# kleinzcy/speech_signal_processing

Hardware: AMD Instinct MI355X
Metric: MFCC frames/s (one fused pass: framing .. DCT + delta + delta-delta, 39-d) (higher is better)
Workload: dtype f32; 1 GPU; configs[1]: 100000 x 3 s synthetic 16 kHz utterances per GPU, 39-d MFCC (+delta+delta-delta), 400/160/512, 24 mel; utterances_per_gpu=100000, frames_per_gpu=29800000, d_out=39, parallelism=utterance-sharded x1, world_size_observed=1

## Files before the change

speech_signal_processing_amd/csrc/cplx.hpp:

```cpp
#pragma once
#include <hip/hip_runtime.h>

namespace ssp {

typedef float v2f __attribute__((ext_vector_type(2)));
typedef float v4f __attribute__((ext_vector_type(4)));
typedef __attribute__((address_space(3))) void* lds_ptr_t;


__device__ __forceinline__ v2f swap(v2f z) { return v2f{z.y, z.x}; }
__device__ __forceinline__ v2f xx(v2f z) { return v2f{z.x, z.x}; }
__device__ __forceinline__ v2f yy(v2f z) { return v2f{z.y, z.y}; }
__device__ __forceinline__ v2f add_neg_i(v2f t, v2f u) { return __builtin_elementwise_fma(swap(u), v2f{1.f, -1.f}, t); }
__device__ __forceinline__ v2f sub_neg_i(v2f t, v2f u) { return __builtin_elementwise_fma(swap(u), v2f{-1.f, 1.f}, t); }
__device__ __forceinline__ v2f cmulc(v2f z, float c, float s) {
    return __builtin_elementwise_fma(yy(z), v2f{-s, c}, xx(z) * v2f{c, s});
}
__device__ __forceinline__ v2f cmul(v2f z, v2f w) {
    v2f t, r;
    asm("v_pk_mul_f32 %0, %1, %2 op_sel_hi:[0,1]" : "=v"(t) : "v"(z), "v"(w));
    asm("v_pk_fma_f32 %0, %1, %2, %3 op_sel:[1,1,0] op_sel_hi:[1,0,1] neg_lo:[0,1,0]"
        : "=v"(r) : "v"(z), "v"(w), "v"(t));
    return r;
}
__device__ __forceinline__ v2f cmul_negi(v2f z, v2f w) {
    v2f t, r;
    asm("v_pk_mul_f32 %0, %1, %2 op_sel:[1,0] op_sel_hi:[1,1]" : "=v"(t) : "v"(z), "v"(w));
    asm("v_pk_fma_f32 %0, %1, %2, %3 op_sel:[0,1,0] op_sel_hi:[0,0,1] neg_hi:[0,1,0]"
        : "=v"(r) : "v"(z), "v"(w), "v"(t));
    return r;
}
__device__ __forceinline__ v2f cmul2(v2f z, v2f w, v2f iw) { return __builtin_elementwise_fma(yy(z), iw, xx(z) * w); }

__device__ __forceinline__ void dft4(v2f& a, v2f& b, v2f& c, v2f& d) {
    const v2f t0 = a + c, t1 = a - c, t2 = b + d, u = b - d;
    a = t0 + t2;
    c = t0 - t2;
    b = add_neg_i(t1, u);
    d = sub_neg_i(t1, u);
}

__device__ __forceinline__ void dft4_d0(v2f& a, v2f& b, v2f& c, v2f& d) {
    const v2f t0 = a + c, t1 = a - c, u = b;
    a = t0 + u;
    c = t0 - u;
    b = add_neg_i(t1, u);
    d = sub_neg_i(t1, u);
}

template <bool TAIL0 = false>
__device__ __forceinline__ void fft16_in(v2f (&z)[16]) {
    constexpr float C1 = 0.92387953251128674f, S1 = 0.38268343236508977f, R = 0.70710678118654752f;
    dft4(z[0], z[4], z[8], z[12]);
#pragma unroll
    for (int n2 = 1; n2 < 4; ++n2) {
        if (TAIL0) dft4_d0(z[n2], z[n2 + 4], z[n2 + 8], z[n2 + 12]);
        else dft4(z[n2], z[n2 + 4], z[n2 + 8], z[n2 + 12]);
    }
    z[5] = cmulc(z[5], C1, -S1);
    z[6] = cmulc(z[6], R, -R);
    z[7] = cmulc(z[7], S1, -C1);
    z[9] = cmulc(z[9], R, -R);
    z[10] = swap(z[10]) * v2f{1.f, -1.f};
    z[11] = cmulc(z[11], -R, -R);
    z[13] = cmulc(z[13], S1, -C1);
    z[14] = cmulc(z[14], -R, -R);
    z[15] = cmulc(z[15], -C1, S1);
#pragma unroll
    for (int k1 = 0; k1 < 4; ++k1) dft4(z[4 * k1], z[4 * k1 + 1], z[4 * k1 + 2], z[4 * k1 + 3]);
    v2f o[16];
#pragma unroll
    for (int k1 = 0; k1 < 4; ++k1)
#pragma unroll
        for (int k2 = 0; k2 < 4; ++k2) o[k1 + 4 * k2] = z[4 * k1 + k2];
#pragma unroll
    for (int i = 0; i < 16; ++i) z[i] = o[i];
}
__device__ __forceinline__ void fft16(v2f (&z)[16]) { fft16_in<false>(z); }

__device__ __forceinline__ void fft8(v2f (&z)[8]) {
    constexpr float R = 0.70710678118654752f;
    dft4(z[0], z[2], z[4], z[6]);
    dft4(z[1], z[3], z[5], z[7]);
    const v2f o0 = z[1], o1 = cmulc(z[3], R, -R), o2 = swap(z[5]) * v2f{1.f, -1.f}, o3 = cmulc(z[7], -R, -R);
    const v2f e0 = z[0], e1 = z[2], e2 = z[4], e3 = z[6];
    z[0] = e0 + o0;
    z[1] = e1 + o1;
    z[2] = e2 + o2;
    z[3] = e3 + o3;
    z[4] = e0 - o0;
    z[5] = e1 - o1;
    z[6] = e2 - o2;
    z[7] = e3 - o3;
}

template <int R>
__device__ __forceinline__ void fft_small(v2f (&z)[R]) {
    if constexpr (R == 2) {
        const v2f a = z[0], b = z[1];
        z[0] = a + b;
        z[1] = a - b;
    } else if constexpr (R == 4) {
        dft4(z[0], z[1], z[2], z[3]);
    } else if constexpr (R == 8) {
        fft8(z);
    } else {
        fft16(z);
    }
}

extern "C" __device__ float ssp_fmul_legacy(float, float) __asm("llvm.amdgcn.fmul.legacy");
__device__ __forceinline__ v2f wmul_edge(v2f y, v2f w) { return v2f{ssp_fmul_legacy(y.x, w.x), ssp_fmul_legacy(y.y, w.y)}; }

__device__ __forceinline__ v2f edge_row_taps(v2f w, int first_tap, int win_len) {
    if (first_tap < win_len && w.x == 0.f) w.x = 1.17549435e-38f;
    if (first_tap + 1 < win_len && w.y == 0.f) w.y = 1.17549435e-38f;
    return w;
}

}
```

speech_signal_processing_amd/csrc/mfcc_stream_kernel.hpp:

```cpp
#pragma once
#include <algorithm>
#include <cmath>
#include <cstdlib>
#include <type_traits>

#include "mfcc.hpp"
#include "cplx.hpp"

namespace ssp {

namespace {
typedef unsigned v2u __attribute__((ext_vector_type(2)));
typedef __attribute__((address_space(3))) const volatile v2f* lds_cv2f_t;
typedef __attribute__((address_space(3))) const volatile float* lds_cvf_t;
typedef __attribute__((address_space(3))) const v2f* lds_c2f_t;
typedef __attribute__((address_space(3))) v4f* lds_4f_t;
constexpr int ZROW = 128;
constexpr int ZFRAME = 16 * ZROW;
constexpr int LM_OFF = 1792;
constexpr int RING_FRAMES = 24;
constexpr int RING_ROW = 64;
constexpr int STREAM_WAVES = 4;
#ifndef SSP_S_PSHIFT
#define SSP_S_PSHIFT 64
#endif
constexpr int PSH = SSP_S_PSHIFT;
static_assert(4 * (256 + 24) + PSH <= LM_OFF - 192, "shifted P row: piece reads must stay below the log-mel rows");
#ifndef SSP_S_NOFLOOR
#define SSP_S_NOFLOOR 1
#endif
#ifndef SSP_S_PUTSC
#define SSP_S_PUTSC 1
#endif
#ifndef SSP_S_AHEAD
#define SSP_S_AHEAD 1
#endif
#ifndef SSP_S_WTAB
#define SSP_S_WTAB 1
#endif
#ifndef SSP_S_LADDR
#define SSP_S_LADDR 1
#endif
constexpr int STREAM_WTAB_N = 39, STREAM_WTAB_BYTES = STREAM_WTAB_N * 8;
constexpr bool stream_wtab(int melv, int ns, int cm, int walk, int geo) { return SSP_S_WTAB && geo >= 2 && !walk && !cm && !(melv >= 4 && ns >= 4); }
#define SSP_STR_(x) #x
#define SSP_STR(x) SSP_STR_(x)

__device__ __forceinline__ float stream_log(const FastArgs& f, float v) {
    return __builtin_amdgcn_logf(fmaxf(v + f.log_add, f.log_max)) * f.log_k;
}

__device__ __forceinline__ float delta_weight(float t, float tp, float Tm1, float half_inv) {
    const float lo = tp <= 0.f ? -1.0e6f : tp;
    const float hi = tp >= Tm1 ? 1.0e6f : tp;
    const float a = fmaxf(lo, t - 2.f), b = fminf(hi, t + 2.f);
    const float cnt = fmaxf(b - a + 1.f, 0.f);
    const float w = cnt * (a + b - 2.f * t) * half_inv;
    return (tp < 0.f || tp > Tm1) ? 0.f : w;
}
}

template <int NZ, int POWER, int PRE, int MELV, int KS, int NS, int OCC, int CM, int WALK, int GEO>
__device__ __forceinline__ void mfcc_stream512_body(const MfccArgs& a, const FastArgs& f, const StreamArgs& sa) {
    static_assert(GEO >= 0 && GEO <= 3 && (GEO == 0 || (NZ == 13 && KS == 6 && MELV != 0)), "fixed geometry: the 400 / 160 / 24-filter family only");
    constexpr bool FIXG = GEO != 0;
    extern __shared__ __attribute__((aligned(16))) char smem[];
    if (WALK && sa.work_counter[1] == 0) return;
    const int tid = threadIdx.x, lane = tid & 63;
    const int wave = __builtin_amdgcn_readfirstlane(tid >> 6);
    const int g = lane >> 4, j = lane & 15;
    constexpr int nc = 13;
    constexpr int mel_ns = NS;

    char* zbuf = smem + wave * sa.wave_bytes;
    float* stage = reinterpret_cast<float*>(zbuf + 4 * ZFRAME);
    char* ring = zbuf + 4 * ZFRAME + sa.stage_bytes;

    v2f wreg[NZ];
#pragma unroll
    for (int n1 = 0; n1 < NZ; ++n1) wreg[n1] = *reinterpret_cast<const v2f*>(a.window + 32 * n1 + 2 * j);
#pragma unroll
    for (int n1 = 0; n1 < NZ; ++n1) wreg[n1] = edge_row_taps(wreg[n1], 32 * n1 + 2 * j, a.win_len);
#ifndef SSP_STREAM_NTW
#define SSP_STREAM_NTW 15
#endif
#ifndef SSP_STREAM_NTW_CM
#define SSP_STREAM_NTW_CM 12
#endif
#ifndef SSP_STREAM_NWP
#define SSP_STREAM_NWP 8
#endif
    constexpr int NTW = OCC >= 3 ? (CM ? SSP_STREAM_NTW_CM : ((MELV <= 3 && NS <= 2) ? SSP_STREAM_NTW : ((MELV >= 4 && NS >= 4) ? 8 : 9))) : 15, NWP = OCC >= 3 ? SSP_STREAM_NWP : 8;
    static_assert(NTW >= 8, "rows above NTW take W^((k1 - 8) j) W^(8 j): W^(8 j) = twr[7] must be resident");
    v2f twr[NTW], wpr[NWP];
#pragma unroll
    for (int k1 = 1; k1 <= NTW; ++k1) twr[k1 - 1] = *reinterpret_cast<const v2f*>(&f.tw16[k1 * 16 + j]);
    float dA[KS];
#pragma unroll
    for (int s = 0; s < KS; ++s) dA[s] = sa.dctA[s * 64 + lane];
#pragma unroll
    for (int i = 0; i < NWP; ++i) wpr[i] = *reinterpret_cast<const v2f*>(&f.wpost[i * 16 + j]);
    constexpr bool DENSE = MELV == 0;
    constexpr int MV = DENSE ? 1 : MELV;
    v4f mw[MV];
    int mofs[MV];
    v2f mk01 = v2f{0.f, 0.f}, mk23 = v2f{0.f, 0.f};
    int mfid = -1;
    v4f dw[DENSE ? 6 : 1][4];
    float dw256[DENSE ? 6 : 1];
    if (DENSE) {
#pragma unroll
        for (int k = 0; k < 6; ++k) {
#pragma unroll
            for (int i = 0; i < 4; ++i) dw[DENSE ? k : 0][i] = *reinterpret_cast<const v4f*>(sa.dense_w + ((size_t)lane * 6 + k) * 20 + 4 * i);
            dw256[DENSE ? k : 0] = sa.dense_w[((size_t)lane * 6 + k) * 20 + 16];
        }
    } else {
#pragma unroll
        for (int i = 0; i < MV; ++i) {
            mw[i] = *reinterpret_cast<const v4f*>(f.pc_w + ((size_t)lane * MV + i) * 4);
            mofs[i] = f.pc_ofs[lane * MV + i];
        }
        mk01 = *reinterpret_cast<const v2f*>(f.pc_mask + lane * 4);
        mk23 = NS > 2 ? *reinterpret_cast<const v2f*>(f.pc_mask + lane * 4 + 2) : v2f{0.f, 0.f};
        mfid = f.pc_fid[lane];
    }

    const int hop = FIXG ? 160 : a.hop;
    const float pre = PRE ? a.preemph : 0.f;
    const float npre = -pre;
    const int slen = FIXG ? 3 * 160 + 32 * 13 : f.slen;
    const int n_piece = (slen + 255) >> 8;
    const bool has_half = (slen & 255) != 0 && (slen & 255) <= 128;
    const int n_full = has_half ? n_piece - 1 : n_piece;
    const int dord = FIXG ? GEO - 1 : a.delta_order;
    const int Dd = FIXG ? nc * GEO : a.d_out;
    const int n_filt = FIXG ? 24 : a.n_filt;
    const int lm_pad = FIXG ? 0 : f.lm_pad;
    const float half_inv = 0.5f * a.delta_inv_denom;
    const uint32_t stage_lds = __builtin_amdgcn_readfirstlane((uint32_t)(uintptr_t)(lds_ptr_t)stage);
    constexpr bool WTAB = FIXG && stream_wtab(MELV, NS, CM, WALK, GEO);
    char* wtab = smem + STREAM_WAVES * sa.wave_bytes;
    if constexpr (WTAB) {
        const float inv = 2.f * half_inv, inv2 = inv * inv;
        const float ds = (float)(lane - 19);
        const float aw = __builtin_fabsf(ds);
        const float w = __builtin_fmaf(aw, __builtin_fmaf(aw * aw, -1.f / 6.f, 37.f / 6.f), -10.f) * inv2;
        if (lane < STREAM_WTAB_N) *reinterpret_cast<v2f*>(wtab + 8 * lane) = v2f{__builtin_fabsf(ds) <= 2.f ? ds * inv : 0.f, aw <= 4.f ? w : 0.f};
        asm volatile("s_waitcnt lgkmcnt(0)" ::: "memory");
    }
    constexpr bool LADDR = FIXG && !WALK && !CM && SSP_S_LADDR;
    int la_dct = 0, la_put = 0, la_pf = 0;
    if constexpr (LADDR) {
        la_dct = (int)(uintptr_t)(lds_ptr_t)(zbuf + (j & 3) * (ZFRAME - 64) + LM_OFF + g * (KS * 4));
        la_put = j < 4 ? (int)(uintptr_t)(lds_ptr_t)(ring + j * RING_ROW + g * 16) : -1;
        la_pf = lane * 16;
        asm volatile("" : "+v"(la_dct), "+v"(la_put), "+v"(la_pf));
    }

#ifdef SSP_S_CLOCK
    const unsigned long long ck0 = __builtin_amdgcn_s_memtime(), rt0 = __builtin_amdgcn_s_memrealtime();
#endif
    uint64_t wm = 0;
    int wblk = blockIdx.x * STREAM_WAVES + wave, wbase = 0;
    constexpr bool AHEAD = FIXG && !WALK && SSP_S_AHEAD;
    typedef int rec_t __attribute__((ext_vector_type(8)));
    int nx_cidx = 0;
    rec_t nx_rec = rec_t{0, 0, 0, 0, 0, 0, 0, 0};
    auto claim_ahead = [&]() {
        const __amdgpu_buffer_rsrc_t rc = __builtin_amdgcn_make_buffer_rsrc(sa.work_counter, 0, 4, 0x00020000);
        int ol = lane;
        asm volatile("" : "+v"(ol));
        const int got = __builtin_amdgcn_raw_ptr_buffer_atomic_add_i32(1, rc, ol == 0 ? 0 : 0x7ffffff0, 0, 0);
        nx_cidx = __builtin_amdgcn_readfirstlane(got);
        const StreamChunkRec* rp = sa.chunk_rec + min(nx_cidx, sa.n_chunks - 1);
        asm volatile("s_load_dwordx8 %0, %1, 0x0\n\ts_waitcnt lgkmcnt(0)" : "=&s"(nx_rec) : "s"(rp) : "memory");
    };
    if constexpr (AHEAD) claim_ahead();
    for (;;) {
        int cidx = 0;
        if constexpr (WALK) {
            bool done = false;
            while (wm == 0) {
                if ((int64_t)wblk * 64 >= sa.n_chunks) {
                    done = true;
                    break;
                }
                const int idx = wblk * 64 + lane;
                const int fl = idx < sa.n_chunks ? sa.redo_flags[idx] : 0;
                wm = __builtin_amdgcn_ballot_w64(fl != 0);
                wbase = wblk * 64;
                wblk += gridDim.x * STREAM_WAVES;
            }
            if (done) break;
            cidx = __builtin_amdgcn_readfirstlane(wbase + __builtin_ctzll(wm));
            wm &= wm - 1;
        } else if constexpr (AHEAD) {
            cidx = nx_cidx;
            if (cidx >= sa.n_chunks) break;
        } else {
            if (lane == 0) cidx = atomicAdd(sa.work_counter, 1);
            cidx = __builtin_amdgcn_readfirstlane(cidx);
            if (cidx >= sa.n_chunks) break;
        }
        MfccChunk ch{};
        int64_t s0, N = 0, f0;
        int T, t0, n, rec_xbytes = 0;
        if constexpr (AHEAD) {
            s0 = (int64_t)(((uint64_t)(uint32_t)nx_rec[1] << 32) | (uint32_t)nx_rec[0]);
            f0 = (int64_t)(((uint64_t)(uint32_t)nx_rec[3] << 32) | (uint32_t)nx_rec[2]);
            rec_xbytes = nx_rec[4];
            T = nx_rec[5];
            t0 = nx_rec[6];
            n = nx_rec[7] & 0xffff;
            ch.pad = nx_rec[7] >> 16;
        } else {
            ch = a.chunks[cidx];
            s0 = a.sample_off[ch.utt];
            N = a.sample_off[ch.utt + 1] - s0;
            f0 = a.frame_off[ch.utt];
            T = __builtin_amdgcn_readfirstlane((int)(a.frame_off[ch.utt + 1] - f0));
            t0 = __builtin_amdgcn_readfirstlane(ch.t0), n = __builtin_amdgcn_readfirstlane(ch.n);
        }
        const int H = dord > 0 ? 4 : 0;
        const int Hlo = dord > 0 ? H + __builtin_amdgcn_readfirstlane(ch.pad) : 0;
        const int ta = max(t0 - Hlo, 0), tb = min(t0 + n + H, T);
        const int R = tb - ta;
        const int nquads = (R + 3) >> 2;
        const int E = t0 + n - ta;
        const int n_steps = (E + 4 + 15) >> 4;
        const int Q = DENSE ? nquads : 4 * n_steps;
        const float Tm1 = (float)(T - 1);

        const uint64_t xaddr = reinterpret_cast<uint64_t>(a.samples + s0);
        const uint32_t xlo = __builtin_amdgcn_readfirstlane((uint32_t)xaddr), xhi = __builtin_amdgcn_readfirstlane((uint32_t)(xaddr >> 32));
        const int xbytes = AHEAD ? rec_xbytes : __builtin_amdgcn_readfirstlane((int)(N * 4));
        const __amdgpu_buffer_rsrc_t rs = __builtin_amdgcn_make_buffer_rsrc(
            reinterpret_cast<float*>(((uint64_t)xhi << 32) | xlo), 0, xbytes, 0x00020000);
        const uint64_t oaddr = reinterpret_cast<uint64_t>(a.out + (size_t)f0 * Dd);
        const uint32_t olo = __builtin_amdgcn_readfirstlane((uint32_t)oaddr), ohi = __builtin_amdgcn_readfirstlane((uint32_t)(oaddr >> 32));
        const __amdgpu_buffer_rsrc_t ro = __builtin_amdgcn_make_buffer_rsrc(
            reinterpret_cast<float*>(((uint64_t)ohi << 32) | olo), 0, __builtin_amdgcn_readfirstlane(T * Dd * 4), 0x00020000);

        auto prefetch = [&](int q) {
            int ol = lane;
            if (FIXG && !LADDR) asm volatile("" : "+v"(ol));
            const int vo = (ta + 4 * q) * hop * 4 + (LADDR ? la_pf : ol * 16);
            const lds_ptr_t lp = (lds_ptr_t)(uintptr_t)stage_lds;
            if (FIXG) {
                __builtin_amdgcn_raw_ptr_buffer_load_lds(rs, lp, 16, vo, 0, 0, 0);
                __builtin_amdgcn_raw_ptr_buffer_load_lds(rs, lp, 16, vo, 0, 1024, 0);
                __builtin_amdgcn_raw_ptr_buffer_load_lds(rs, lp, 16, vo, 0, 2048, 0);
                if (LADDR ? la_pf < 512 : lane < 32) __builtin_amdgcn_raw_ptr_buffer_load_lds(rs, lp, 16, vo, 0, 3072, 0);
                return;
            }
            if (n_full > 0) __builtin_amdgcn_raw_ptr_buffer_load_lds(rs, lp, 16, vo, 0, 0, 0);
            if (n_full > 1) __builtin_amdgcn_raw_ptr_buffer_load_lds(rs, lp, 16, vo, 0, 1024, 0);
            if (n_full > 2) __builtin_amdgcn_raw_ptr_buffer_load_lds(rs, lp, 16, vo, 0, 2048, 0);
            if (n_full > 3) __builtin_amdgcn_raw_ptr_buffer_load_lds(rs, lp, 16, vo, 0, 3072, 0);
            if (n_full > 4) __builtin_amdgcn_raw_ptr_buffer_load_lds(rs, (lds_ptr_t)(uintptr_t)(stage_lds + 4096), 16, vo + 4096, 0, 0, 0);
            if (has_half && lane < 32)
                __builtin_amdgcn_raw_ptr_buffer_load_lds(rs, (lds_ptr_t)(uintptr_t)(stage_lds + n_full * 1024), 16, vo + n_full * 1024, 0, 0, 0);
        };

        {
            float zz = 0.f;
            asm volatile("" : "+v"(zz));
            v4f z4 = v4f{zz, zz, zz, zz};
            *reinterpret_cast<v4f*>(ring + lane * 16) = z4;
            if (lane < (RING_FRAMES * RING_ROW - 1024) / 16) *reinterpret_cast<v4f*>(ring + 1024 + lane * 16) = z4;
        }
        prefetch(0);
        int stores_pending = 0;
        int cm_nf = WALK;
        float cs1[CM ? 3 : 1] = {}, cs2[CM ? 3 : 1] = {};
        float piv = 0.f;

        typedef v2f zarr_t[16];
        typedef v2f pfarr_t[NZ];
        typedef float pmarr_t[PRE ? NZ : 1];
        constexpr int NH = (NZ + 1) / 2;
        auto wait_dma = [&]() {
#ifndef SSP_S_NOWAIT
            if constexpr (FIXG) {
                if (__builtin_expect(stores_pending == 0, 1)) {
                    asm volatile("s_waitcnt vmcnt(0)" ::: "memory");
                } else {
                    int np = stores_pending;
                    asm volatile("" : "+s"(np));
                    if (np == 2 * GEO) asm volatile("s_waitcnt vmcnt(%0)" ::"n"(2 * GEO) : "memory");
                    else asm volatile("s_waitcnt vmcnt(%0)" ::"n"(GEO >= 3 ? 13 : (GEO == 2 ? 9 : 4)) : "memory");
                }
            } else {
                if (stores_pending == 0) asm volatile("s_waitcnt vmcnt(0)" ::: "memory");
                else if (stores_pending == 2) asm volatile("s_waitcnt vmcnt(2)" ::: "memory");
                else if (stores_pending == 4) asm volatile("s_waitcnt vmcnt(4)" ::: "memory");
                else if (stores_pending == 6) asm volatile("s_waitcnt vmcnt(6)" ::: "memory");
                else if (stores_pending == 9) asm volatile("s_waitcnt vmcnt(9)" ::: "memory");
                else asm volatile("s_waitcnt vmcnt(13)" ::: "memory");
            }
#endif
            stores_pending = 0;
        };
        auto stage_read_a = [&](pfarr_t& pf, pmarr_t& pm) {
            const uint32_t sp = stage_lds + (g * hop + 2 * j) * 4;
#pragma unroll
            for (int n1 = 0; n1 < NH; ++n1) {
                pf[n1] = *(lds_cv2f_t)(uintptr_t)(sp + 128 * n1);
#ifdef SSP_S_PM64
                if (PRE) pm[n1] = (*(lds_cv2f_t)(uintptr_t)(sp + 128 * n1 - 8)).y;
#else
                if (PRE) pm[n1] = *(lds_cvf_t)(uintptr_t)(sp + 128 * n1 - 4);
#endif
            }
        };
        auto stage_read_b = [&](pfarr_t& pf, pmarr_t& pm) {
            const uint32_t sp = stage_lds + (g * hop + 2 * j) * 4;
#pragma unroll
            for (int n1 = NH; n1 < NZ; ++n1) {
                pf[n1] = *(lds_cv2f_t)(uintptr_t)(sp + 128 * n1);
#ifdef SSP_S_PM64
                if (PRE) pm[n1] = (*(lds_cv2f_t)(uintptr_t)(sp + 128 * n1 - 8)).y;
#else
                if (PRE) pm[n1] = *(lds_cvf_t)(uintptr_t)(sp + 128 * n1 - 4);
#endif
            }
        };
        auto win_rows = [&](zarr_t& z, pfarr_t& pf, pmarr_t& pm, auto lo_tag, auto hi_tag, auto edge_tag) {
            constexpr int LO = decltype(lo_tag)::value, HI = decltype(hi_tag)::value;
            constexpr int EDGE = decltype(edge_tag)::value;
#pragma unroll
            for (int n1 = LO; n1 < HI; ++n1) {
                if (n1 < NZ) {
                    v2f y = pf[n1 < NZ ? n1 : 0];
                    if (PRE) {
                        const float xm1 = pm[n1 < NZ ? n1 : 0], x0 = y.x, x1 = y.y;
                        y = v2f{__builtin_fmaf(npre, xm1, x0), __builtin_fmaf(npre, x0, x1)};
                    }
                    z[n1] = (EDGE == 1 || (EDGE == 2 && n1 == NZ - 1)) ? wmul_edge(y, wreg[n1 < NZ ? n1 : 0]) : y * wreg[n1 < NZ ? n1 : 0];
                } else {
                    z[n1] = v2f{0.f, 0.f};
                }
            }
        };
        auto window_a = [&](zarr_t& z, pfarr_t& pf, pmarr_t& pm, auto edge_tag) {
            if (PRE) pm[0] = (j == 0) ? pf[0].x : pm[0];
            win_rows(z, pf, pm, std::integral_constant<int, 0>{}, std::integral_constant<int, NH>{}, edge_tag);
        };
        auto window_b = [&](zarr_t& z, pfarr_t& pf, pmarr_t& pm, auto edge_tag) {
            win_rows(z, pf, pm, std::integral_constant<int, NH>{}, std::integral_constant<int, 16>{}, edge_tag);
        };
        auto fft_front = [&](zarr_t& z) {
            fft16_in<(NZ <= 13)>(z);
#pragma unroll
            for (int k1 = 1; k1 < 16; ++k1) {
                if (k1 <= NTW) {
                    z[k1] = cmul(z[k1], twr[(k1 - 1) % NTW]);
                } else {
                    z[k1] = cmul(cmul(z[k1], twr[(k1 - 9) % NTW]), twr[7]);
                }
            }
            char* zf = zbuf + g * ZFRAME;
            {
                int wb0 = ((j >> 1) << 4) | ((j & 1) << 3);
                asm volatile("" : "+v"(wb0));
#pragma unroll
                for (int m = 0; m < 8; ++m) {
                    char* wp = zf + (wb0 ^ (m << 4));
                    *reinterpret_cast<v2f*>(wp + (2 * m) * ZROW) = z[2 * m];
                    *reinterpret_cast<v2f*>(wp + (2 * m + 1) * ZROW) = z[2 * m + 1];
                }
                int rb0 = j * ZROW + (((j >> 1) & 7) << 4);
                asm volatile("" : "+v"(rb0));
#pragma unroll
                for (int c = 0; c < 8; ++c) {
                    const v4f r = *reinterpret_cast<const v4f*>(zf + (rb0 ^ (c << 4)));
                    z[2 * c] = v2f{r.x, r.y};
                    z[2 * c + 1] = v2f{r.z, r.w};
                }
            }
            fft16(z);
            {
                float* P = reinterpret_cast<float*>(zf + (PSH ? (g & 1) * PSH : 0));
                float* Pm = P + 144 - j;
#pragma unroll
                for (int kp = 0; kp < 4; ++kp) {
                    v2f e[2], d[2], w[2];
#pragma unroll
                    for (int u = 0; u < 2; ++u) {
                        const int k2 = 2 * kp + u;
                        const float sx = z[15 - k2].x, sy = z[15 - k2].y;
                        const v2f own = z[(16 - k2) & 15];
                        const float ox = own.x, oy = own.y;
                        float mx = __builtin_amdgcn_update_dpp(sx, sx, 0x140 , 0xF, 0xF, true);
                        float my = __builtin_amdgcn_update_dpp(sy, sy, 0x140 , 0xF, 0xF, true);
                        mx = __builtin_amdgcn_update_dpp(ox, mx, 0x111 , 0xF, 0xF, false);
                        my = __builtin_amdgcn_update_dpp(oy, my, 0x111 , 0xF, 0xF, false);
                        const v2f zmk = v2f{mx, my};
                        const v2f zk = z[k2];
                        w[u] = wpr[k2 < NWP ? k2 : k2 - 4];
                        if (k2 >= NWP) w[u] = cmulc(w[u], 0.70710678118654752f, -0.70710678118654752f);
                        e[u] = __builtin_elementwise_fma(zmk, v2f{1.f, -1.f}, zk);
                        d[u] = __builtin_elementwise_fma(zmk, v2f{-1.f, 1.f}, zk);
                    }
                    d[0] = cmul_negi(d[0], w[0]);
                    d[1] = cmul_negi(d[1], w[1]);
                    float pa[2], pb[2];
#pragma unroll
                    for (int u = 0; u < 2; ++u) {
                        const v2f o = d[u];
                        const v2f Rr = __builtin_elementwise_fma(xx(o), v2f{1.f, -1.f}, xx(e[u]));
                        const v2f Ii = __builtin_elementwise_fma(yy(o), v2f{1.f, -1.f}, yy(e[u]));
                        const v2f pw = __builtin_elementwise_fma(Rr, Rr, Ii * Ii);
                        pa[u] = pw.x;
                        pb[u] = pw.y;
                        if (POWER == 1) {
                            pa[u] = __builtin_amdgcn_sqrtf(pa[u]);
                            pb[u] = __builtin_amdgcn_sqrtf(pb[u]);
                        }
                    }
                    const int k2 = 2 * kp;
                    P[j + 16 * k2] = pa[0];
                    P[j + 16 * (k2 + 1)] = pa[1];
                    Pm[16 * (6 - k2)] = pb[1];
                    Pm[16 * (7 - k2)] = pb[0];
                }
                const v2f s8 = z[8] * z[8];
                float p128 = 4.f * (s8.x + s8.y);
                if (POWER == 1) p128 = __builtin_amdgcn_sqrtf(p128);
                if (j == 0) P[128] = p128;
            }
        };
        auto mel = [&]() {
#ifndef SSP_S_NOMEL
            if (!CM) {
                float* lm = reinterpret_cast<float*>(zbuf + g * ZFRAME + LM_OFF - 64 * g);
                if (j < lm_pad) lm[n_filt + j] = 0.f;
            } else if (j < lm_pad) {
                int ol = lane;
                asm volatile("" : "+v"(ol));
                reinterpret_cast<float*>(zbuf + (ol >> 4) * (ZFRAME - 64) + LM_OFF)[n_filt + (ol & 15)] = 0.f;
            }
            float sfr[4];
#pragma unroll
            for (int fr = 0; fr < 4; ++fr) {
                const char* pr = zbuf + fr * ZFRAME + (fr & 1) * PSH;
                v4f acc = *reinterpret_cast<const v4f*>(pr + mofs[0]) * mw[0];
#pragma unroll
                for (int i = 1; i < MV; ++i) acc = __builtin_elementwise_fma(*reinterpret_cast<const v4f*>(pr + mofs[i]), mw[i], acc);
                const v2f h = v2f{acc.x, acc.y} + v2f{acc.z, acc.w};
                sfr[fr] = h.x + h.y;
            }
            v2f s01 = v2f{sfr[0], sfr[1]}, s23 = v2f{sfr[2], sfr[3]};
#define SSP_SCAN_STEP(CTRL, MK)                                                                     \
            {                                                                                           \
                const float a0 = s01.x, a1 = s01.y, a2 = s23.x, a3 = s23.y;                             \
                const float b0 = __builtin_amdgcn_update_dpp(a0, a0, CTRL, 0xF, 0xF, true);           \
                const float b1 = __builtin_amdgcn_update_dpp(a1, a1, CTRL, 0xF, 0xF, true);           \
                const float b2 = __builtin_amdgcn_update_dpp(a2, a2, CTRL, 0xF, 0xF, true);           \
                const float b3 = __builtin_amdgcn_update_dpp(a3, a3, CTRL, 0xF, 0xF, true);           \
                s01 = __builtin_elementwise_fma(v2f{b0, b1}, MK, s01);                                  \
                s23 = __builtin_elementwise_fma(v2f{b2, b3}, MK, s23);                                  \
            }
            if (mel_ns > 0) SSP_SCAN_STEP(0x101 , xx(mk01))
            if (mel_ns > 1) SSP_SCAN_STEP(0x102 , yy(mk01))
            if (mel_ns > 2) SSP_SCAN_STEP(0x104 , xx(mk23))
            if (mel_ns > 3) SSP_SCAN_STEP(0x108 , yy(mk23))
#undef SSP_SCAN_STEP
            auto slog = [&](float v) -> float {
                if constexpr (FIXG && SSP_S_NOFLOOR) return __builtin_amdgcn_logf(v) * f.log_k;
                else return stream_log(f, v);
            };
            if (mfid >= 0) {
                float* lmf = reinterpret_cast<float*>(zbuf + LM_OFF) + mfid;
                lmf[0 * (ZFRAME - 64) / 4] = slog(s01.x);
                lmf[1 * (ZFRAME - 64) / 4] = slog(s01.y);
                lmf[2 * (ZFRAME - 64) / 4] = slog(s23.x);
                lmf[3 * (ZFRAME - 64) / 4] = slog(s23.y);
            }
#endif
        };
        auto dct_mfma = [&]() -> v4f {
            v4f cq = v4f{0.f, 0.f, 0.f, 0.f};
#ifndef SSP_S_NODCT
            int ol = lane;
            if (!LADDR) asm volatile("" : "+v"(ol));
            const int g = ol >> 4, j = ol & 15;
            const char* lmrow = zbuf + (j & 3) * (ZFRAME - 64) + LM_OFF + g * (KS * 4);
            float lb[KS];
#pragma unroll
            for (int s = 0; s < KS; s += 2) {
                const v2f v = LADDR ? *(lds_c2f_t)(uintptr_t)(uint32_t)(la_dct + 4 * s) : *reinterpret_cast<const v2f*>(lmrow + 4 * s);
                lb[s] = v.x;
                lb[s + 1] = v.y;
            }
#pragma unroll
            for (int s = 0; s < KS; ++s) cq = __builtin_amdgcn_mfma_f32_16x16x4f32(dA[s], lb[s], cq, 0, 0, 0);
#endif
            return cq;
        };
        constexpr int RING_BYTES = RING_FRAMES * RING_ROW, QROW = 4 * RING_ROW;
        auto ring_wrap = [](int o) { return o >= RING_BYTES ? o - RING_BYTES : o; };
        int qrow = 0, srow = 0;
        auto ring_put = [&](int qq, v4f cq, bool real) {
            int ol = lane;
            asm volatile("" : "+v"(ol));
            const int g = ol >> 4, j = ol & 15;
            if (j < 4) {
                const bool ok = real && ta + 4 * qq + j < tb;
                const v4f cv = ok ? cq : v4f{0.f, 0.f, 0.f, 0.f};
                if constexpr (FIXG) *reinterpret_cast<v4f*>(ring + qrow + j * RING_ROW + g * 16) = cv;
                else *reinterpret_cast<v4f*>(ring + ((((qq + 6) % 6) * 4 + j) * RING_ROW) + g * 16) = cv;
            }
            if (FIXG) qrow = ring_wrap(qrow + QROW);
        };
        auto ring_put_inner = [&](v4f cq, bool on) {
            int ol = lane;
            asm volatile("" : "+v"(ol));
            const int g = ol >> 4, j = ol & 15;
            if constexpr (LADDR) {
                if (la_put >= 0 && on) *(lds_4f_t)(uintptr_t)(uint32_t)(la_put + qrow) = cq;
            } else {
                if (j < 4 && on) *reinterpret_cast<v4f*>(ring + qrow + j * RING_ROW + g * 16) = cq;
            }
            qrow = ring_wrap(qrow + QROW);
        };
        typedef float cbarr_t[6];
        auto ring_window = [&](int b, cbarr_t& cb) {
            const int rb = 16 * b;
            int ol = lane;
            asm volatile("" : "+v"(ol));
            const int g = ol >> 4, j = ol & 15;
            int mb = ring_wrap(srow + 16 * RING_ROW);
#pragma unroll
            for (int s = 0; s < 6; ++s) {
                if constexpr (FIXG) {
                    cb[s] = *reinterpret_cast<const float*>(ring + mb + g * RING_ROW + j * 4);
                    mb = ring_wrap(mb + QROW);
                } else {
                    const int m = (rb + 16 + 4 * s) % RING_FRAMES;
                    cb[s] = *reinterpret_cast<const float*>(ring + (m + g) * RING_ROW + j * 4);
                }
            }
        };
        auto time_step = [&](int b, const cbarr_t& cb) {
            const int rb = 16 * b;
            int ol = lane;
            asm volatile("" : "+v"(ol));
            const int g = ol >> 4, j = ol & 15;
            const float tg = (float)(ta + rb);
            const bool interior = ta + rb - 8 >= 1 && ta + rb + 16 <= T - 2;
            const float inv = 2.f * half_inv;
            auto W = [&](float tr, float tpr) -> float {
                if (interior) {
                    const float d = tpr - tr;
                    return __builtin_fabsf(d) <= 2.f ? d * inv : 0.f;
                }
                return delta_weight(tg + tr, tg + tpr, Tm1, half_inv);
            };
            const float fj = (float)j, fg = (float)g;
            const int Fo = ta + rb - 4 + 4 * g;
            const bool full = ta + rb - 4 >= t0 && ta + rb + 12 <= t0 + n;
            const int lane_off = j < nc ? (Fo * Dd + j) * 4 : 0x7ffffff0;
            auto put = [&](int rrel, int blk, float v, bool lane_on) {
                int off;
                if (full) {
                    off = lane_on ? lane_off + (rrel * Dd + blk * nc) * 4 : 0x7ffffff0;
                } else {
                    const int F = Fo + rrel;
                    off = (lane_on && F >= t0 && F < t0 + n) ? lane_off + (rrel * Dd + blk * nc) * 4 : 0x7ffffff0;
                }
#ifdef SSP_S_NOSTORE
                asm volatile("" ::"v"(v), "v"(off));
#else
                __builtin_amdgcn_raw_buffer_store_b32(__builtin_bit_cast(unsigned, v), ro, off, 0, 0);
#endif
                if (CM) {
                    const float dv = off != 0x7ffffff0 ? (blk == 0 ? v - piv : v) : 0.f;
                    cs1[CM ? blk : 0] += dv;
                    cs2[CM ? blk : 0] = __builtin_fmaf(dv, dv, cs2[CM ? blk : 0]);
                }
            };
            if (CM && b == 0) piv = j < nc ? *reinterpret_cast<const float*>(ring + j * 4) : 0.f;
            {
                const float* cr;
                if constexpr (FIXG) {
                    const int slot = ring_wrap(ring_wrap(srow + 20 * RING_ROW) + 4 * g * RING_ROW);
                    cr = reinterpret_cast<const float*>(ring + slot + j * 4);
                } else {
                    const int m4 = (rb + 20) % RING_FRAMES;
                    int slot = m4 + 4 * g;
                    slot = slot >= RING_FRAMES ? slot - RING_FRAMES : slot;
                    cr = reinterpret_cast<const float*>(ring + slot * RING_ROW + j * 4);
                }
                const v4f o0 = v4f{cr[0], cr[16], cr[32], cr[48]};
#pragma unroll
                for (int r = 0; r < 4; ++r) put(r, 0, o0[r], true);
            }
            if (dord >= 1) {
                v4f d0 = v4f{0.f, 0.f, 0.f, 0.f}, d1 = v4f{0.f, 0.f, 0.f, 0.f};
#pragma unroll
                for (int s = 0; s < 5; ++s) d0 = __builtin_amdgcn_mfma_f32_16x16x4f32(W(fj - 6.f, fg + (float)(4 * s - 8)), cb[s], d0, 0, 0, 0);
                const float fr1 = (float)(j >> 2) + 10.f;
#pragma unroll
                for (int s = 4; s < 6; ++s) {
                    float w = W(fr1, fg + (float)(4 * s - 8));
                    w = (j & 3) == 0 ? w : 0.f;
                    d1 = __builtin_amdgcn_mfma_f32_16x16x4f32(w, cb[s], d1, 0, 0, 0);
                }
#pragma unroll
                for (int r = 0; r < 4; ++r) put(r - 2, 1, d0[r], r >= 2 || g > 0);
                put(14 - 3 * g, 1, d1[0], g < 2);
                if (dord >= 2) {
                    v4f dd = v4f{0.f, 0.f, 0.f, 0.f};
#pragma unroll
                    for (int s = 0; s < 4; ++s) dd = __builtin_amdgcn_mfma_f32_16x16x4f32(W(fj - 4.f, 4.f * fg + (float)(s - 6)), d0[s], dd, 0, 0, 0);
                    dd = __builtin_amdgcn_mfma_f32_16x16x4f32(W(fj - 4.f, fg + 10.f), d1[0], dd, 0, 0, 0);
#pragma unroll
                    for (int r = 0; r < 4; ++r) put(r, 2, dd[r], true);
                }
            }
            stores_pending = dord >= 2 ? 13 : (dord == 1 ? 9 : 4);
        };
        auto time_step_T = [&](int b, const cbarr_t& cb) {
            const int rb = 16 * b;
            int ol = lane;
            asm volatile("" : "+v"(ol));
            const int g = ol >> 4, j = ol & 15;
            const float inv = 2.f * half_inv;
            const float ef = (float)(g - 4 - j);
            const int F = ta + rb - 4 + j;
            const bool emit = F >= t0 && F < t0 + n;
            const int row16 = (emit && g < 3) ? (F * Dd + 4 * g) * 4 : 0x7ffffff0;
            const int row4 = (emit && g == 3) ? (F * Dd + 12) * 4 : 0x7ffffff0;
            auto store = [&](v4f v, int blk) {
                typedef unsigned v4u_t __attribute__((ext_vector_type(4)));
                __builtin_amdgcn_raw_buffer_store_b128(__builtin_bit_cast(v4u_t, v), ro, row16 + blk * (nc * 4), 0, 0);
                __builtin_amdgcn_raw_buffer_store_b32(__builtin_bit_cast(unsigned, v.x), ro, row4 + blk * (nc * 4), 0, 0);
            };
            {
                v4f c;
                if constexpr (FIXG) {
                    const int slot = ring_wrap(ring_wrap(srow + 20 * RING_ROW) + j * RING_ROW);
                    c = *reinterpret_cast<const v4f*>(ring + slot + g * 16);
                } else {
                    int slot = (rb + 20) % RING_FRAMES + j;
                    slot = slot >= RING_FRAMES ? slot - RING_FRAMES : slot;
                    c = *reinterpret_cast<const v4f*>(ring + slot * RING_ROW + g * 16);
                }
                store(c, 0);
            }
            v2f wt[6] = {};
            if constexpr (WTAB) {
                const char* wl = wtab + 8 * (g - j + 15);
#pragma unroll
                for (int s = 0; s < 6; ++s) {
                    if constexpr (GEO >= 3) wt[s] = *reinterpret_cast<const v2f*>(wl + 32 * s);
                    else wt[s].x = *reinterpret_cast<const float*>(wl + 32 * s);
                }
            }
            if (dord >= 1) {
                v4f d = v4f{0.f, 0.f, 0.f, 0.f};
#pragma unroll
                for (int s = 0; s < 6; ++s) {
                    const float ds = ef + (float)(4 * s);
                    d = __builtin_amdgcn_mfma_f32_16x16x4f32(cb[s], WTAB ? wt[s].x : (__builtin_fabsf(ds) <= 2.f ? ds * inv : 0.f), d, 0, 0, 0);
                }
                store(d, 1);
            }
            if (dord >= 2) {
                v4f q = v4f{0.f, 0.f, 0.f, 0.f};
                const float inv2 = inv * inv;
#pragma unroll
                for (int s = 0; s < 6; ++s) {
                    const float a = __builtin_fabsf(ef + (float)(4 * s));
                    const float w = __builtin_fmaf(a, __builtin_fmaf(a * a, -1.f / 6.f, 37.f / 6.f), -10.f) * inv2;
                    q = __builtin_amdgcn_mfma_f32_16x16x4f32(cb[s], WTAB ? wt[s].y : (a <= 4.f ? w : 0.f), q, 0, 0, 0);
                }
                store(q, 2);
            }
            stores_pending = 2 * (1 + dord);
        };
        auto time_step_nf = [&](int b) {
            const int rb = 16 * b;
            int ol = lane;
            asm volatile("" : "+v"(ol));
            const int g = ol >> 4, j = ol & 15;
            const float inv = 2.f * half_inv;
            const int F = ta + rb - 4 + j;
            const bool emit = F >= t0 && F < t0 + n;
#pragma unroll 1
            for (int k = 0; k < 4; ++k) {
                const int col = 4 * g + k;
                const int off = (emit && col < nc) ? (F * Dd + col) * 4 : 0x7ffffff0;
                auto cread = [&](int t) -> float {
                    t = min(max(t, 0), T - 1);
                    const unsigned slot = (unsigned)(t - ta + 2 * RING_FRAMES) % (unsigned)RING_FRAMES;
                    return *reinterpret_cast<const float*>(ring + slot * RING_ROW + col * 4);
                };
                auto dl = [&](int u) -> float {
                    u = min(max(u, 0), T - 1);
                    float s = 0.f;
#pragma unroll 1
                    for (int m = -2; m <= 2; ++m) s = __builtin_fmaf((float)m, cread(u + m), s);
                    return s * inv;
                };
                auto store = [&](float v, int blk) { __builtin_amdgcn_raw_buffer_store_b32(__builtin_bit_cast(unsigned, v), ro, off + blk * (nc * 4), 0, 0); };
                store(cread(F), 0);
                if (dord >= 1) store(dl(F), 1);
                if (dord >= 2) {
                    float q = 0.f;
#pragma unroll 1
                    for (int kk = -2; kk <= 2; ++kk) q = __builtin_fmaf((float)kk, dl(F + kk), q);
                    store(q * inv, 2);
                }
            }
            stores_pending = 0;
            cm_nf = 1;
        };
        auto emit_step = [&](int b) {
            cbarr_t cb;
            ring_window(b, cb);
#ifdef SSP_S_NOTSTEP
            time_step(b, cb);
#else
            const bool interior = ta + 16 * b - 8 >= 1 && ta + 16 * b + 16 <= T - 2;
            constexpr bool TSTEP = !CM && !(MELV >= 4 && NS >= 4);
            if (TSTEP && interior) time_step_T(b, cb);
            else time_step(b, cb);
#endif
            if (FIXG) srow = ring_wrap(srow + 16 * RING_ROW);
        };

        if constexpr (DENSE) {
            static_assert(!(DENSE && WALK), "the dense-band instance has no time steps: nothing to walk again");
            for (int q = 0; q < nquads; ++q) {
                zarr_t z;
                pfarr_t pf;
                pmarr_t pm;
                wait_dma();
                stage_read_a(pf, pm);
                asm volatile("s_waitcnt lgkmcnt(0)" ::: "memory");
                window_a(z, pf, pm, std::integral_constant<int, DENSE ? 2 : 0>{});
                stage_read_b(pf, pm);
                asm volatile("s_waitcnt lgkmcnt(0)" ::: "memory");
#ifndef SSP_S_NODMA
                prefetch(q + 1);
#endif
                window_b(z, pf, pm, std::integral_constant<int, DENSE ? 2 : 0>{});
                fft_front(z);
                int ol = lane;
                asm volatile("" : "+v"(ol));
                const int c = ol & 15;
                float r[4][6];
#pragma unroll
                for (int fr = 0; fr < 4; ++fr) {
                    const char* pr = zbuf + fr * ZFRAME + (fr & 1) * PSH;
                    const v4f p0 = *reinterpret_cast<const v4f*>(pr + 64 * c), p1 = *reinterpret_cast<const v4f*>(pr + 64 * c + 16);
                    const v4f p2 = *reinterpret_cast<const v4f*>(pr + 64 * c + 32), p3 = *reinterpret_cast<const v4f*>(pr + 64 * c + 48);
                    const float p256 = *reinterpret_cast<const float*>(pr + 1024);
#pragma unroll
                    for (int k = 0; k < 6; ++k) {
                        v4f acc = p0 * dw[DENSE ? k : 0][0];
                        acc = __builtin_elementwise_fma(p1, dw[DENSE ? k : 0][1], acc);
                        acc = __builtin_elementwise_fma(p2, dw[DENSE ? k : 0][2], acc);
                        acc = __builtin_elementwise_fma(p3, dw[DENSE ? k : 0][3], acc);
                        const v2f hs = v2f{acc.x, acc.y} + v2f{acc.z, acc.w};
                        r[fr][k] = __builtin_fmaf(p256, dw256[DENSE ? k : 0], hs.x + hs.y);
                    }
                }
                float* sc = reinterpret_cast<float*>(zbuf);
#pragma unroll
                for (int fr = 0; fr < 4; ++fr)
#pragma unroll
                    for (int k = 0; k < 6; ++k) sc[(fr * 6 + k) * 64 + ol] = r[fr][k];
                const int nb = a.n_filt;
#pragma unroll
                for (int rd = 0; rd < 2; ++rd) {
                    const int o = rd * 64 + ol;
                    const int fr = (o >= nb) + (o >= 2 * nb) + (o >= 3 * nb);
                    const int band = o - fr * nb;
                    const int bg = (band * 43) >> 8, k = band - 6 * bg;
                    const bool valid = o < 4 * nb;
                    const float* src = sc + ((valid ? fr * 6 + k : 0) * 64 + (valid ? 16 * bg : 0));
                    const v4f s0 = *reinterpret_cast<const v4f*>(src), s1 = *reinterpret_cast<const v4f*>(src + 4);
                    const v4f s2 = *reinterpret_cast<const v4f*>(src + 8), s3 = *reinterpret_cast<const v4f*>(src + 12);
                    const v4f s4 = (s0 + s1) + (s2 + s3);
                    const float val = stream_log(f, (s4.x + s4.y) + (s4.z + s4.w));
                    const bool ok = valid && ta + 4 * q + fr < tb;
                    __builtin_amdgcn_raw_buffer_store_b32(__builtin_bit_cast(unsigned, val), ro, ok ? ((ta + 4 * q) * Dd + o) * 4 : 0x7ffffff0, 0, 0);
                }
                asm volatile("s_waitcnt lgkmcnt(0)" ::: "memory");
                stores_pending = 2;
            }
        } else if constexpr (WALK) {
            for (int q = 0; q < Q; ++q) {
                if (q < nquads) {
                    zarr_t z;
                    pfarr_t pf;
                    pmarr_t pm;
                    wait_dma();
                    stage_read_a(pf, pm);
                    asm volatile("s_waitcnt lgkmcnt(0)" ::: "memory");
                    window_a(z, pf, pm, std::integral_constant<int, 1>{});
                    stage_read_b(pf, pm);
                    asm volatile("s_waitcnt lgkmcnt(0)" ::: "memory");
                    prefetch(q + 1);
                    window_b(z, pf, pm, std::integral_constant<int, 1>{});
                    fft_front(z);
                    mel();
                    const v4f cq = dct_mfma();
                    ring_put(q, cq, true);
                } else {
                    ring_put(q, v4f{0.f, 0.f, 0.f, 0.f}, false);
                }
                if ((q & 3) == 3) time_step_nf(q >> 2);
            }
        } else {
#ifdef SSP_S_SEQ
            for (int q = 0; q < Q; ++q) {
                zarr_t z;
                pfarr_t pf;
                pmarr_t pm;
                if (q < nquads) {
                    wait_dma();
                    stage_read_a(pf, pm);
                    asm volatile("s_waitcnt lgkmcnt(0)" ::: "memory");
                    window_a(z, pf, pm, std::integral_constant<int, DENSE ? 2 : 0>{});
                    stage_read_b(pf, pm);
                    asm volatile("s_waitcnt lgkmcnt(0)" ::: "memory");
#ifndef SSP_S_NODMA
                    prefetch(q + 1);
#endif
                    window_b(z, pf, pm, std::integral_constant<int, DENSE ? 2 : 0>{});
                    fft_front(z);
                    mel();
                    const v4f cq = dct_mfma();
                    ring_put(q, cq, true);
                } else {
                    ring_put(q, v4f{0.f, 0.f, 0.f, 0.f}, false);
                }
#ifndef SSP_S_NOSTEP
                if ((q & 3) == 3) emit_step(q >> 2);
#endif
            }
#else
#ifdef SSP_S_PAD
            asm volatile(".rept " SSP_STR(SSP_S_PAD) "\n s_nop 0\n .endr");
#endif
            if (FIXG) qrow = 5 * QROW;
            for (int q = 0; q < nquads; ++q) {
                zarr_t z;
                pfarr_t pf;
                pmarr_t pm;
                wait_dma();
                stage_read_a(pf, pm);
                const v4f cq = dct_mfma();
                asm volatile("s_waitcnt lgkmcnt(0)" ::: "memory");
                window_a(z, pf, pm, std::integral_constant<int, DENSE ? 2 : 0>{});
                stage_read_b(pf, pm);
                if constexpr (FIXG && SSP_S_PUTSC) ring_put_inner(cq, q > 0);
                else ring_put(q - 1, cq, q > 0);
                asm volatile("s_waitcnt lgkmcnt(0)" ::: "memory");
#ifndef SSP_S_NODMA
                prefetch(q + 1);
#endif
                window_b(z, pf, pm, std::integral_constant<int, DENSE ? 2 : 0>{});
                fft_front(z);
                mel();
#ifndef SSP_S_NOSTEP
                if ((q & 3) == 0 && q > 0) emit_step((q - 1) >> 2);
#endif
            }
            for (int qb = nquads - 1; qb < Q; ++qb) {
                v4f cq = v4f{0.f, 0.f, 0.f, 0.f};
                if (qb < nquads) cq = dct_mfma();
                ring_put(qb, cq, qb < nquads);
#ifndef SSP_S_NOSTEP
                if ((qb & 3) == 3) emit_step(qb >> 2);
#endif
            }
#endif
        }
        if constexpr (AHEAD) claim_ahead();
// ... 255 lines not shown
```

Measured before the change: 3.302 billion frames/s.

## Precompute FFT constant pairs in SGPRs and hoist per-step LDS/store address math

Constant sign and twiddle pairs for the radix-16 FFT are materialised once as scalar-register pairs and passed into an FFT variant, so each packed FMA no longer rebuilds its inline literal vector. Per-lane LDS base addresses for the ring window and delta-weight table are computed once, and a ring offset is advanced each step, replacing per-step modular slot arithmetic. Output row offsets use a 24-bit multiply. Log-mel writes from inactive lanes are redirected to a junk slot so the branch on the filter index goes away. The aim is fewer VALU and address instructions in the hot loop, at the cost of extra live registers and more complex address bookkeeping.

```diff
diff --git a/speech_signal_processing_amd/csrc/cplx.hpp b/speech_signal_processing_amd/csrc/cplx.hpp
--- a/speech_signal_processing_amd/csrc/cplx.hpp
+++ b/speech_signal_processing_amd/csrc/cplx.hpp
@@ -78,6 +78,57 @@
 }
 __device__ __forceinline__ void fft16(v2f (&z)[16]) { fft16_in<false>(z); }
 
+struct Fft16Pairs {
+    v2f pm, mp;
+    v2f c1s1, s1c1;
+    v2f c1ms1, s1mc1;
+    v2f mc1s1, ms1mc1;
+    v2f rr, rmr;
+};
+__device__ __forceinline__ void dft4_k(v2f& a, v2f& b, v2f& c, v2f& d, const Fft16Pairs& k) {
+    const v2f t0 = a + c, t1 = a - c, t2 = b + d, u = b - d;
+    a = t0 + t2;
+    c = t0 - t2;
+    b = __builtin_elementwise_fma(swap(u), k.pm, t1);
+    d = __builtin_elementwise_fma(swap(u), k.mp, t1);
+}
+__device__ __forceinline__ void dft4_d0_k(v2f& a, v2f& b, v2f& c, v2f& d, const Fft16Pairs& k) {
+    const v2f t0 = a + c, t1 = a - c, u = b;
+    a = t0 + u;
+    c = t0 - u;
+    b = __builtin_elementwise_fma(swap(u), k.pm, t1);
+    d = __builtin_elementwise_fma(swap(u), k.mp, t1);
+}
+__device__ __forceinline__ v2f cmulk(v2f z, v2f A, v2f B) { return __builtin_elementwise_fma(yy(z), A, xx(z) * B); }
+template <bool TAIL0 = false>
+__device__ __forceinline__ void fft16_in_k(v2f (&z)[16], const Fft16Pairs& k) {
+    constexpr float R = 0.70710678118654752f;
+    dft4_k(z[0], z[4], z[8], z[12], k);
+#pragma unroll
+    for (int n2 = 1; n2 < 4; ++n2) {
+        if (TAIL0) dft4_d0_k(z[n2], z[n2 + 4], z[n2 + 8], z[n2 + 12], k);
+        else dft4_k(z[n2], z[n2 + 4], z[n2 + 8], z[n2 + 12], k);
+    }
+    z[5] = cmulk(z[5], k.s1c1, k.c1ms1);
+    z[6] = cmulk(z[6], k.rr, k.rmr);
+    z[7] = cmulk(z[7], k.c1s1, k.s1mc1);
+    z[9] = cmulk(z[9], k.rr, k.rmr);
+    z[10] = swap(z[10]) * k.pm;
+    z[11] = cmulk(z[11], k.rmr, v2f{-R, -R});
+    z[13] = cmulk(z[13], k.c1s1, k.s1mc1);
+    z[14] = cmulk(z[14], k.rmr, v2f{-R, -R});
+    z[15] = cmulk(z[15], k.ms1mc1, k.mc1s1);
+#pragma unroll
+    for (int k1 = 0; k1 < 4; ++k1) dft4_k(z[4 * k1], z[4 * k1 + 1], z[4 * k1 + 2], z[4 * k1 + 3], k);
+    v2f o[16];
+#pragma unroll
+    for (int k1 = 0; k1 < 4; ++k1)
+#pragma unroll
+        for (int k2 = 0; k2 < 4; ++k2) o[k1 + 4 * k2] = z[4 * k1 + k2];
+#pragma unroll
+    for (int i = 0; i < 16; ++i) z[i] = o[i];
+}
+
 __device__ __forceinline__ void fft8(v2f (&z)[8]) {
     constexpr float R = 0.70710678118654752f;
     dft4(z[0], z[2], z[4], z[6]);
diff --git a/speech_signal_processing_amd/csrc/mfcc_stream_kernel.hpp b/speech_signal_processing_amd/csrc/mfcc_stream_kernel.hpp
--- a/speech_signal_processing_amd/csrc/mfcc_stream_kernel.hpp
+++ b/speech_signal_processing_amd/csrc/mfcc_stream_kernel.hpp
@@ -41,6 +41,19 @@
 #ifndef SSP_S_LADDR
 #define SSP_S_LADDR 1
 #endif
+#ifndef SSP_S_KPAIR
+#define SSP_S_KPAIR 1
+#endif
+#ifndef SSP_S_JUNK
+#define SSP_S_JUNK 1
+#endif
+#ifndef SSP_S_STEPADDR
+#define SSP_S_STEPADDR 1
+#endif
+#ifndef SSP_S_LADDR_CM
+#define SSP_S_LADDR_CM 1
+#endif
+constexpr bool stream_junk(int cm, int walk, int geo) { return SSP_S_JUNK && SSP_S_LADDR && geo >= 1 && !walk && !cm; }
 constexpr int STREAM_WTAB_N = 39, STREAM_WTAB_BYTES = STREAM_WTAB_N * 8;
 constexpr bool stream_wtab(int melv, int ns, int cm, int walk, int geo) { return SSP_S_WTAB && geo >= 2 && !walk && !cm && !(melv >= 4 && ns >= 4); }
 #define SSP_STR_(x) #x
@@ -149,13 +162,45 @@
         if (lane < STREAM_WTAB_N) *reinterpret_cast<v2f*>(wtab + 8 * lane) = v2f{__builtin_fabsf(ds) <= 2.f ? ds * inv : 0.f, aw <= 4.f ? w : 0.f};
         asm volatile("s_waitcnt lgkmcnt(0)" ::: "memory");
     }
-    constexpr bool LADDR = FIXG && !WALK && !CM && SSP_S_LADDR;
+    constexpr bool LADDR = FIXG && !WALK && (!CM || SSP_S_LADDR_CM) && SSP_S_LADDR;
+    constexpr bool JUNK = LADDR && stream_junk(CM, WALK, GEO);
     int la_dct = 0, la_put = 0, la_pf = 0;
     if constexpr (LADDR) {
         la_dct = (int)(uintptr_t)(lds_ptr_t)(zbuf + (j & 3) * (ZFRAME - 64) + LM_OFF + g * (KS * 4));
         la_put = j < 4 ? (int)(uintptr_t)(lds_ptr_t)(ring + j * RING_ROW + g * 16) : -1;
         la_pf = lane * 16;
         asm volatile("" : "+v"(la_dct), "+v"(la_put), "+v"(la_pf));
+    }
+    int mfid_j = mfid;
+    if constexpr (JUNK) {
+        mfid_j = mfid >= 0 ? mfid : 4 * KS;
+        asm volatile("" : "+v"(mfid_j));
+    }
+    constexpr bool STEPADDR = LADDR && !CM && SSP_S_STEPADDR;
+    constexpr bool STEPWT = STEPADDR && WTAB;
+    int la_rw = 0, la_wt = 0;
+    if constexpr (STEPADDR) {
+        la_rw = (int)(uintptr_t)(lds_ptr_t)(ring + g * RING_ROW + j * 4);
+        asm volatile("" : "+v"(la_rw));
+        if constexpr (STEPWT) {
+            la_wt = (int)(uintptr_t)(lds_ptr_t)(wtab + 8 * (g - j + 15));
+            asm volatile("" : "+v"(la_wt));
+        }
+    }
+    constexpr bool KPAIR = FIXG && !WALK && !CM && SSP_S_KPAIR;
+    Fft16Pairs kc{};
+    if constexpr (KPAIR) {
+        constexpr float C1 = 0.92387953251128674f, S1 = 0.38268343236508977f, R = 0.70710678118654752f;
+        auto pair = [](float lo, float hi) {
+            v2f p = v2f{lo, hi};
+            asm volatile("" : "+s"(p));
+            return p;
+        };
+        kc.pm = pair(1.f, -1.f), kc.mp = pair(-1.f, 1.f);
+        kc.c1s1 = pair(C1, S1), kc.s1c1 = pair(S1, C1);
+        kc.c1ms1 = pair(C1, -S1), kc.s1mc1 = pair(S1, -C1);
+        kc.mc1s1 = pair(-C1, S1), kc.ms1mc1 = pair(-S1, -C1);
+        kc.rr = pair(R, R), kc.rmr = pair(R, -R);
     }
 
 #ifdef SSP_S_CLOCK
@@ -351,7 +396,8 @@
             win_rows(z, pf, pm, std::integral_constant<int, NH>{}, std::integral_constant<int, 16>{}, edge_tag);
         };
         auto fft_front = [&](zarr_t& z) {
-            fft16_in<(NZ <= 13)>(z);
+            if constexpr (KPAIR) fft16_in_k<(NZ <= 13)>(z, kc);
+            else fft16_in<(NZ <= 13)>(z);
 #pragma unroll
             for (int k1 = 1; k1 < 16; ++k1) {
                 if (k1 <= NTW) {
@@ -379,7 +425,8 @@
                     z[2 * c + 1] = v2f{r.z, r.w};
                 }
             }
-            fft16(z);
+            if constexpr (KPAIR) fft16_in_k<false>(z, kc);
+            else fft16(z);
             {
                 float* P = reinterpret_cast<float*>(zf + (PSH ? (g & 1) * PSH : 0));
                 float* Pm = P + 144 - j;
@@ -400,8 +447,8 @@
                         const v2f zk = z[k2];
                         w[u] = wpr[k2 < NWP ? k2 : k2 - 4];
                         if (k2 >= NWP) w[u] = cmulc(w[u], 0.70710678118654752f, -0.70710678118654752f);
-                        e[u] = __builtin_elementwise_fma(zmk, v2f{1.f, -1.f}, zk);
-                        d[u] = __builtin_elementwise_fma(zmk, v2f{-1.f, 1.f}, zk);
+                        e[u] = __builtin_elementwise_fma(zmk, KPAIR ? kc.pm : v2f{1.f, -1.f}, zk);
+                        d[u] = __builtin_elementwise_fma(zmk, KPAIR ? kc.mp : v2f{-1.f, 1.f}, zk);
                     }
                     d[0] = cmul_negi(d[0], w[0]);
                     d[1] = cmul_negi(d[1], w[1]);
@@ -409,8 +456,8 @@
 #pragma unroll
                     for (int u = 0; u < 2; ++u) {
                         const v2f o = d[u];
-                        const v2f Rr = __builtin_elementwise_fma(xx(o), v2f{1.f, -1.f}, xx(e[u]));
-                        const v2f Ii = __builtin_elementwise_fma(yy(o), v2f{1.f, -1.f}, yy(e[u]));
+                        const v2f Rr = __builtin_elementwise_fma(xx(o), KPAIR ? kc.pm : v2f{1.f, -1.f}, xx(e[u]));
+                        const v2f Ii = __builtin_elementwise_fma(yy(o), KPAIR ? kc.pm : v2f{1.f, -1.f}, yy(e[u]));
                         const v2f pw = __builtin_elementwise_fma(Rr, Rr, Ii * Ii);
                         pa[u] = pw.x;
                         pb[u] = pw.y;
@@ -471,8 +518,8 @@
                 if constexpr (FIXG && SSP_S_NOFLOOR) return __builtin_amdgcn_logf(v) * f.log_k;
                 else return stream_log(f, v);
             };
-            if (mfid >= 0) {
-                float* lmf = reinterpret_cast<float*>(zbuf + LM_OFF) + mfid;
+            if (JUNK || mfid >= 0) {
+                float* lmf = reinterpret_cast<float*>(zbuf + LM_OFF) + (JUNK ? mfid_j : mfid);
                 lmf[0 * (ZFRAME - 64) / 4] = slog(s01.x);
                 lmf[1 * (ZFRAME - 64) / 4] = slog(s01.y);
                 lmf[2 * (ZFRAME - 64) / 4] = slog(s23.x);
@@ -502,6 +549,7 @@
         constexpr int RING_BYTES = RING_FRAMES * RING_ROW, QROW = 4 * RING_ROW;
         auto ring_wrap = [](int o) { return o >= RING_BYTES ? o - RING_BYTES : o; };
         int qrow = 0, srow = 0;
+        int mrow = 16 * RING_ROW;
         auto ring_put = [&](int qq, v4f cq, bool real) {
             int ol = lane;
             asm volatile("" : "+v"(ol));
@@ -516,7 +564,7 @@
         };
         auto ring_put_inner = [&](v4f cq, bool on) {
             int ol = lane;
-            asm volatile("" : "+v"(ol));
+            if (!JUNK) asm volatile("" : "+v"(ol));
             const int g = ol >> 4, j = ol & 15;
             if constexpr (LADDR) {
                 if (la_put >= 0 && on) *(lds_4f_t)(uintptr_t)(uint32_t)(la_put + qrow) = cq;
@@ -528,6 +576,18 @@
         typedef float cbarr_t[6];
         auto ring_window = [&](int b, cbarr_t& cb) {
             const int rb = 16 * b;
+            if constexpr (STEPADDR) {
+                static_assert(RING_FRAMES == 24 && QROW == 4 * RING_ROW, "the window of a step covers the ring exactly once");
+                const int m1 = mrow >= 16 * RING_ROW ? mrow - RING_BYTES : mrow, m2 = mrow >= 8 * RING_ROW ? mrow - RING_BYTES : mrow;
+                const uint32_t a0 = (uint32_t)(la_rw + mrow), a1 = (uint32_t)(la_rw + m1), a2 = (uint32_t)(la_rw + m2);
+                cb[0] = *(lds_cvf_t)(uintptr_t)(a0);
+                cb[1] = *(lds_cvf_t)(uintptr_t)(a0 + QROW);
+                cb[2] = *(lds_cvf_t)(uintptr_t)(a1 + 2 * QROW);
+                cb[3] = *(lds_cvf_t)(uintptr_t)(a1 + 3 * QROW);
+                cb[4] = *(lds_cvf_t)(uintptr_t)(a2 + 4 * QROW);
+                cb[5] = *(lds_cvf_t)(uintptr_t)(a2 + 5 * QROW);
+                return;
+            }
             int ol = lane;
             asm volatile("" : "+v"(ol));
             const int g = ol >> 4, j = ol & 15;
@@ -631,8 +691,9 @@
             const float ef = (float)(g - 4 - j);
             const int F = ta + rb - 4 + j;
             const bool emit = F >= t0 && F < t0 + n;
-            const int row16 = (emit && g < 3) ? (F * Dd + 4 * g) * 4 : 0x7ffffff0;
-            const int row4 = (emit && g == 3) ? (F * Dd + 12) * 4 : 0x7ffffff0;
+            const int frow = STEPADDR ? (ta + rb - 4) * (Dd * 4) + (int)__umul24((unsigned)j, (unsigned)(Dd * 4)) : 0;
+            const int row16 = (emit && g < 3) ? (STEPADDR ? frow + 4 * g * 4 : (F * Dd + 4 * g) * 4) : 0x7ffffff0;
+            const int row4 = (emit && g == 3) ? (STEPADDR ? frow + 12 * 4 : (F * Dd + 12) * 4) : 0x7ffffff0;
             auto store = [&](v4f v, int blk) {
                 typedef unsigned v4u_t __attribute__((ext_vector_type(4)));
                 __builtin_amdgcn_raw_buffer_store_b128(__builtin_bit_cast(v4u_t, v), ro, row16 + blk * (nc * 4), 0, 0);
@@ -652,11 +713,17 @@
             }
             v2f wt[6] = {};
             if constexpr (WTAB) {
+                typedef __attribute__((address_space(3))) const float* lds_cf_t;
                 const char* wl = wtab + 8 * (g - j + 15);
 #pragma unroll
                 for (int s = 0; s < 6; ++s) {
-                    if constexpr (GEO >= 3) wt[s] = *reinterpret_cast<const v2f*>(wl + 32 * s);
-                    else wt[s].x = *reinterpret_cast<const float*>(wl + 32 * s);
+                    if constexpr (STEPWT) {
+                        if constexpr (GEO >= 3) wt[s] = *(lds_c2f_t)(uintptr_t)(uint32_t)(la_wt + 32 * s);
+                        else wt[s].x = *(lds_cf_t)(uintptr_t)(uint32_t)(la_wt + 32 * s);
+                    } else {
+                        if constexpr (GEO >= 3) wt[s] = *reinterpret_cast<const v2f*>(wl + 32 * s);
+                        else wt[s].x = *reinterpret_cast<const float*>(wl + 32 * s);
+                    }
                 }
             }
             if (dord >= 1) {
@@ -730,6 +797,7 @@
             else time_step(b, cb);
 #endif
             if (FIXG) srow = ring_wrap(srow + 16 * RING_ROW);
+            if (STEPADDR) mrow = ring_wrap(mrow + 16 * RING_ROW);
         };
 
         if constexpr (DENSE) {
```

New measurement: 3.306 billion frames/s, median of 2. About the same (+0.1%).
